# hwwang55/GraphGAN

Measured on AMD Instinct MI355X. Metric: sampled_edges_per_sec, higher is better.
Workload: dtype f32

## Files before the change

### graphgan_amd/_lib.py

```python
from __future__ import annotations

import ctypes
import os

_HERE = os.path.dirname(os.path.abspath(__file__))
LIB_PATH = os.path.join(_HERE, "libgraphgan_hip.so")
HEADER_PATH = os.path.join(os.path.dirname(_HERE), "include", "graphgan_hip.h")
ABI_VERSION = 9


def header_abi_version(path=HEADER_PATH):
    import re
    with open(path) as f:
        m = re.search(r"^#define\s+GG_ABI_VERSION\s+(\d+)", f.read(), flags=re.M)
    if not m:
        raise RuntimeError("GG_ABI_VERSION not found in %s" % path)
    return int(m.group(1))

GG_OK, GG_EINVAL, GG_ECAPACITY, GG_EHIP, GG_ECOMM, GG_ENOMEM, GG_EIO = 0, -1, -2, -3, -4, -5, -6
GG_OPT_ADAM_DENSE, GG_OPT_ADAM_LAZY, GG_OPT_SGD = 0, 1, 2
GG_ROOT_OK, GG_ROOT_ABORTED, GG_ROOT_EMPTY = 0, 1, 2
GG_GS_FOR_D, GG_GS_Q3_STORE = 1, 2
ERROR_NAMES = {GG_EINVAL: "GG_EINVAL", GG_ECAPACITY: "GG_ECAPACITY", GG_EHIP: "GG_EHIP", GG_ECOMM: "GG_ECOMM",
               GG_ENOMEM: "GG_ENOMEM", GG_EIO: "GG_EIO"}


class GGConfig(ctypes.Structure):
    _fields_ = [("lr_gen", ctypes.c_float), ("lr_dis", ctypes.c_float),
                ("lambda_gen", ctypes.c_float), ("lambda_dis", ctypes.c_float),
                ("adam_beta1", ctypes.c_float), ("adam_beta2", ctypes.c_float), ("adam_eps", ctypes.c_float),
                ("window_size", ctypes.c_int32), ("optimizer", ctypes.c_int32), ("device", ctypes.c_int32),
                ("reserved", ctypes.c_int32 * 6)]


class GGCounters(ctypes.Structure):
    _fields_ = [("walks", ctypes.c_int64), ("hops", ctypes.c_int64), ("nbr_reads", ctypes.c_int64),
                ("reward_pairs", ctypes.c_int64), ("d_pairs", ctypes.c_int64), ("g_pairs", ctypes.c_int64),
                ("d_steps", ctypes.c_int64), ("g_steps", ctypes.c_int64),
                ("last_kernel_ms", ctypes.c_double), ("walk_kernel_ms", ctypes.c_double),
                ("walk_launches", ctypes.c_int64), ("rows_scored", ctypes.c_int64), ("score_kernel_ms", ctypes.c_double),
                ("score_launches", ctypes.c_int64), ("score_chunks", ctypes.c_int64), ("score_rows", ctypes.c_int64),
                ("bfs_kernel_ms", ctypes.c_double), ("bfs_trees", ctypes.c_int64), ("score_dists", ctypes.c_int64),
                ("reward_kernel_ms", ctypes.c_double), ("reward_pairs_timed", ctypes.c_int64),
                ("d_grad_ms", ctypes.c_double), ("d_opt_ms", ctypes.c_double), ("d_pairs_timed", ctypes.c_int64), ("d_rows_timed", ctypes.c_int64),
                ("g_grad_ms", ctypes.c_double), ("g_opt_ms", ctypes.c_double), ("g_pairs_timed", ctypes.c_int64), ("g_rows_timed", ctypes.c_int64),
                ("d_passes_timed", ctypes.c_int64), ("g_passes_timed", ctypes.c_int64),
                ("g_walk_nodes_timed", ctypes.c_int64),
                ("es_gathers", ctypes.c_int64), ("es_nodes", ctypes.c_int64), ("score_gathers", ctypes.c_int64), ("score_nodes", ctypes.c_int64),
                ("walk_reruns", ctypes.c_int64)]


class GGGraph(ctypes.Structure):
    _fields_ = [("n_node", ctypes.c_int32), ("nnz", ctypes.c_int64), ("n_train_edges", ctypes.c_int64),
                ("n_test_edges", ctypes.c_int64), ("rowptr", ctypes.POINTER(ctypes.c_int64)), ("col", ctypes.POINTER(ctypes.c_int32))]


class GraphGANHipError(RuntimeError):
    def __init__(self, code, msg):
        super().__init__("%s (%d): %s" % (ERROR_NAMES.get(code, "GG_E?"), code, msg))
        self.code = code


_P = ctypes.c_void_p
_i32, _i64, _u32, _u64 = ctypes.c_int32, ctypes.c_int64, ctypes.c_uint32, ctypes.c_uint64

SIGNATURES = {
    "gg_abi_version": (ctypes.c_int, []),
    "gg_last_error": (ctypes.c_char_p, [_P]),
    "gg_create": (ctypes.c_int, [_i32, _i32, _P, _P, ctypes.POINTER(GGConfig), ctypes.POINTER(_P)]),
    "gg_destroy": (ctypes.c_int, [_P]),
    "gg_set_graph_csr": (ctypes.c_int, [_P, _P, _P]),
    "gg_host_build_trees": (_i64, [_i32, _P, _P, _P, _i32, _P, _P, _P, _i64, _i32, _P]),
    "gg_build_trees": (ctypes.c_int, [_P, _P, _i32, _i32]),
    "gg_build_trees_device": (ctypes.c_int, [_P, _P, _i32]),
    "gg_set_tree_mode": (ctypes.c_int, [_P, _i32, _i64]),
    "gg_debug_words": (ctypes.c_int, [_P, _i32, _i32, _P]),
    "gg_lazy_stats": (ctypes.c_int, [_P, _P]),
    "gg_get_lazy_trees": (ctypes.c_int, [_P, _P, _P, _P, _P, _P, _P, _P]),
    "gg_set_trees": (ctypes.c_int, [_P, _P, _i32, _P, _P, _P, _i32]),
    "gg_tree_info": (ctypes.c_int, [_P, _P, _P, _P]),
    "gg_tree_roots": (ctypes.c_int, [_P, _P]),
    "gg_save_trees": (ctypes.c_int, [_P, ctypes.c_char_p]),
# ... 84 lines not shown
```

### graphgan_amd/csrc/epoch.hip

```cpp
#include <algorithm>
#include <vector>

#include "gg_internal.h"

namespace gg {

int launch_pair_reward(gg_ctx *ctx, const int32_t *d_u, const int32_t *d_v, int64_t n, float *d_out);

__global__ __launch_bounds__(256) void q3_copy_kernel(const int32_t *t_root, const int64_t *t_q3off, uint32_t *t_q3, const int64_t *s_off,
                                                      uint32_t *store, int n_slots, int to_store) {
    const int s = blockIdx.x * blockDim.x + threadIdx.x;
    if (s >= n_slots) return;
    const int v = t_root[s];
    const int64_t a = t_q3off[s], b = s_off[v], words = min(t_q3off[s + 1] - a, s_off[v + 1] - b);
    for (int64_t k = 0; k < words; ++k) {
        if (to_store) store[b + k] = t_q3[a + k];
        else t_q3[a + k] = store[b + k];
    }
}

static int ensure_q3_store(gg_ctx *ctx) {
    if (ctx->q3_store_ready) return GG_OK;
    GG_CHECK(ctx, !ctx->h_rowptr.empty(), GG_EINVAL, "epoch: call gg_set_graph_csr first");
    const int n = ctx->n_node;
// ... 96 lines not shown
        if (rc == GG_OK && do_g) {
            int64_t pairs = 0;
            rc = gg_prepare_g(ctx, slots.data(), n_roots, n_sample, seed, stream_g, &pairs, nullptr);
            if (rc == GG_OK) rc = ensure_g_pairs(ctx);
            if (rc == GG_OK) rc = append(ctx, ctx->ep_node1, ctx->g_node1, ctx->ep_pairs, pairs, sizeof(int32_t));
            if (rc == GG_OK) rc = append(ctx, ctx->ep_node2, ctx->g_node2, ctx->ep_pairs, pairs, sizeof(int32_t));
            if (rc == GG_OK) ctx->ep_pairs += pairs;
        }
        ctx->in_epoch_add = false;
        if (rc != GG_OK) return rc;
        GG_HIP(ctx, hipStreamSynchronize(ctx->stream));
    }
    if (rows_total_out) *rows_total_out = ctx->ep_rows;
    if (pairs_total_out) *pairs_total_out = ctx->ep_pairs;
    return GG_OK;
}

int gg_epoch_commit(gg_ctx *ctx, int32_t which, int64_t *n_out) {
    if (!ctx) return fail(nullptr, GG_EINVAL, "ctx is NULL");
    GG_CHECK(ctx, which == 0 || which == 1, GG_EINVAL, "gg_epoch_commit: which must be 0 (generator pairs) or 1 (discriminator rows)");
    GG_HIP(ctx, hipSetDevice(ctx->device));
    discard_begun_walk(ctx);
    GG_HIP(ctx, hipStreamSynchronize(ctx->stream));
    int rc;
    if (which == 1) {
        const int64_t rows = ctx->ep_rows;
        GG_HIP(ctx, ctx->ep_center.reserve(sizeof(int32_t)));
        GG_HIP(ctx, ctx->ep_neighbor.reserve(sizeof(int32_t)));
        GG_HIP(ctx, ctx->ep_label.reserve(sizeof(float)));
        std::swap(ctx->d_center, ctx->ep_center);
        std::swap(ctx->d_neighbor, ctx->ep_neighbor);
        std::swap(ctx->d_label, ctx->ep_label);
        ctx->d_rows = rows;
        ctx->ep_rows = 0;
        ctx->ep_d_open = false;
        rc = exchange_count_max(ctx, ctx->d_rows, &ctx->d_rows_max);
        if (rc != GG_OK) return rc;
        if (n_out) *n_out = rows;
    } else {
        const int64_t pairs = ctx->ep_pairs;
        GG_HIP(ctx, ctx->ep_node1.reserve(sizeof(int32_t)));
        GG_HIP(ctx, ctx->ep_node2.reserve(sizeof(int32_t)));
        GG_HIP(ctx, ctx->ep_reward.reserve(sizeof(float) * (size_t)(pairs + 1)));
        rc = launch_pair_reward(ctx, ctx->ep_node1.as<int32_t>(), ctx->ep_node2.as<int32_t>(), pairs, ctx->ep_reward.as<float>());
        if (rc != GG_OK) return rc;
        GG_HIP(ctx, hipStreamSynchronize(ctx->stream));
        std::swap(ctx->g_node1, ctx->ep_node1);
        std::swap(ctx->g_node2, ctx->ep_node2);
        std::swap(ctx->g_reward, ctx->ep_reward);
        ctx->g_pairs = pairs;
        ctx->g_pairs_filled = true;
        ctx->g_paths_valid = false;
        ctx->ep_pairs = 0;
        rc = exchange_count_max(ctx, ctx->g_pairs, &ctx->g_pairs_max);
        if (rc != GG_OK) return rc;
        if (n_out) *n_out = pairs;
    }
    return GG_OK;
}

int gg_q3_clear(gg_ctx *ctx) {
    if (!ctx) return fail(nullptr, GG_EINVAL, "ctx is NULL");
    GG_HIP(ctx, hipSetDevice(ctx->device));
    int rc = ensure_q3_store(ctx);
    if (rc != GG_OK) return rc;
    GG_HIP(ctx, hipStreamSynchronize(ctx->stream));
// ... 17 lines not shown
```

### graphgan_amd/csrc/gg_internal.h

```cpp
#pragma once
#include <hip/hip_runtime.h>
#include <stdint.h>
#include <stdio.h>
#include <string>
#include <vector>

#include "../../include/graphgan_hip.h"

namespace gg {

struct DevBuf {
    void *p = nullptr;
    size_t bytes = 0;
    hipError_t reserve(size_t need) {
        if (need <= bytes) return hipSuccess;
        if (p) {
            (void)hipDeviceSynchronize();
            (void)hipFree(p);
        }
        p = nullptr;
        bytes = 0;
        size_t want = need + need / 4 + 256;
        hipError_t e = hipMalloc(&p, want);
        if (e == hipSuccess) bytes = want;
// ... 135 lines not shown
    int tm_cur = -1;

    gg::DevBuf d_center, d_neighbor, d_label, d_cnt, d_ptr;
    int64_t d_rows = 0;
    gg::DevBuf g_node1, g_node2, g_reward, g_cnt, g_ptr;
    int64_t g_pairs = 0;
    bool g_paths_valid = false;
    bool g_begun = false;
    struct { int32_t n_slots = 0, n_sample = 0; uint64_t seed = 0; uint32_t stream = 0; } g_begun_args;
    gg::DevBuf touched_ptr;
    gg::DevBuf bfs_key, bfs_bm, bfs_misc, bfs_sparse, bfs_rowptr32;
    bool bfs_rowptr32_valid = false;
    gg::DevBuf q3_store, q3s_off;
    int64_t q3_words = 0;
    bool q3_store_ready = false;
    gg::DevBuf ep_center, ep_neighbor, ep_label, ep_node1, ep_node2, ep_reward;
    int64_t ep_rows = 0, ep_pairs = 0;
    std::vector<int32_t> ep_slots;
    bool in_epoch_add = false;
    int n_cus = 256;
    gg::DevBuf scan_tmp, step_u, step_v, step_x;
    gg::DevBuf sg_cnt, sg_off, sg_slot, sg_list, sg_rows, sg_bias, sg_tot, sg_key;
    bool g_pairs_filled = false;
    bool sg_cnt_dirty = false;
    gg::DevBuf sgp_cnt, sgp_off, sgp_slot, sgp_list, sgp_tot, sgp_key, sgp_scan, sgp_hub;
    gg::DevBuf sg_hub, hub_acc;
    int64_t hub_cap = 0;
    hipEvent_t ev_slots_done = nullptr;
    bool g_slots_ready = false;
    bool sgp_cnt_clean = false;
    int g_slots_unused = 0;
    int64_t g_slots_walks = 0;
    int32_t g_slots_stride = 0;
    int32_t *sg_cnt_active = nullptr;
    bool sg_active = false;
    int sg_threshold = 64;

    unsigned long long *dev_ctr = nullptr;
    gg_counters ctr{};

    void *comm = nullptr;
    bool comm_rsag = true;
    size_t grad_elems_padded = 0;
    int64_t d_rows_max = 0, g_pairs_max = 0;
    int64_t step_bound = 0;
    int64_t comm_steps_sparse = 0, comm_steps_dense = 0, comm_bytes_sent = 0;
    int32_t rank = 0, world = 1;
    bool deterministic = true;
    float dense_exchange_ratio = 1.5f;
    int32_t fake_world = 0;
    gg::DevBuf x_cnt, x_send_ids, x_send_rows, x_recv_ids, x_recv_rows;
    gg::DevBuf x_nglob;
    gg::DevBuf x_own;
    int32_t owner_exchange = 1;
    bool comm_bf16 = false;
    int64_t owner_min_bound = 4096;
    int64_t comm_steps_owner = 0;

    gg::DevBuf topk_adj;
    bool topk_adj_valid = false;

    gg::DevBuf gs_es, gs_cpre;
    int64_t gs_chunks = 0;
    bool gs_es_valid = false, gs_cpre_valid = false;

    gg::DevBuf pt_starts, pt_paths, pt_len, pt_cnt, pt_ptr, pt_noise, pt_sample;
// ... 23 lines not shown
#define GG_CHECK(ctx, cond, code, ...)                        \
    do {                                                      \
        if (!(cond)) return gg::fail(ctx, code, __VA_ARGS__); \
    } while (0)

int device_exclusive_scan(gg_ctx *ctx, const int32_t *cnt, int64_t *ptr, int64_t n);
int ensure_g_pairs(gg_ctx *ctx);
int device_compact_flags(gg_ctx *ctx, const int32_t *flag, int64_t n, int32_t *list, int64_t *total_out);
int device_segment_rows(gg_ctx *ctx, const int32_t *cnt, int64_t n, int T, int32_t *off, int4 *list, int64_t *totals, hipStream_t stream = nullptr,
                        DevBuf *scratch = nullptr);

int alloc_trees(gg_ctx *ctx, const int32_t *roots, int32_t n_roots, const int64_t *node_counts, const int64_t *root_children, int64_t extra_nodes = 0);
bool lazy_build_wanted(const gg_ctx *ctx);
int lazy_rebuild_whole(gg_ctx *ctx);
int lazy_fallback_rebuild(gg_ctx *ctx, int *n_out);
void component_sizes(int n, const int64_t *rowptr, const int32_t *col, std::vector<int32_t> &comp_size);
int32_t host_bfs_order(const int64_t *rowptr, const int32_t *col, int32_t root, int32_t *order, int32_t *cstart,
                       std::vector<uint32_t> &stamp, uint32_t &epoch, int32_t *depth_out, int32_t *max_children_out);
void order_to_lists(int32_t n, int32_t C, const int32_t *order, const int32_t *cstart, const uint32_t *q3, int32_t *off, int32_t *nbr);
int32_t lists_to_order(int32_t n, int32_t root, const int32_t *off, const int32_t *nbr, int32_t *order, int32_t *cstart,
                       uint32_t *q3, int32_t q3_words, int32_t *depth_out, int32_t *max_children_out);

int walk_launch_async(gg_ctx *ctx, const int32_t *slots, const int32_t *n_walks, int32_t uniform_walks, int32_t n_slots,
                      int32_t for_d, uint64_t seed, uint32_t stream, int32_t stride, bool side_stream = false, bool defer_join = false);
void discard_begun_walk(gg_ctx *ctx);
int walk_finalize(gg_ctx *ctx, bool *retried);
int timing_slot(gg_ctx *ctx);
int check_exchange_flag(gg_ctx *ctx);
void harvest_timings(gg_ctx *ctx);
int derive_tree_edges(gg_ctx *ctx);
int compute_reverse_edges(gg_ctx *ctx);
int rescan_table_finite(gg_ctx *ctx, int which);
int enqueue_path_slots(gg_ctx *ctx);
void generator_changed(gg_ctx *ctx);
int walk_resident(gg_ctx *ctx, const int32_t *slots, const int32_t *n_walks, int32_t uniform_walks, int32_t n_slots,
                  int32_t for_d, uint64_t seed, uint32_t stream, int32_t stride);
int launch_walk_sample(gg_ctx *ctx, int32_t n_slots, int64_t total_walks, int for_d, uint64_t seed, uint32_t stream,
                       int32_t stride);
int run_step(gg_ctx *ctx, int which, const int32_t *d_u, const int32_t *d_v, const float *d_x, int32_t n);
int comm_allreduce_grads(gg_ctx *ctx);
int comm_allreduce_flags(gg_ctx *ctx);
int comm_allreduce_i64(gg_ctx *ctx, int64_t *buf, size_t count);
int comm_allreduce_max_i64(gg_ctx *ctx, int64_t *buf, size_t count);
size_t comm_dense_bytes(const gg_ctx *ctx);
int exchange_count_max(gg_ctx *ctx, int64_t local, int64_t *max_out);
int comm_allgather(gg_ctx *ctx, const void *send, void *recv, size_t count, int elem_bytes);
bool comm_has_p2p(const gg_ctx *ctx);
int comm_exchange_v(gg_ctx *ctx, const float *send, const int64_t *send_off, const int64_t *send_cnt, float *recv, const int64_t *recv_off,
                    const int64_t *recv_cnt);
void comm_destroy(gg_ctx *ctx);

static inline int cdiv(int64_t a, int64_t b) { return (int)((a + b - 1) / b); }

}
```

### graphgan_amd/csrc/prepare.hip

```cpp
#include <algorithm>

#include <cstring>

#include "gg_internal.h"

namespace gg {

constexpr int SCAN_THREADS = 256;
constexpr int SCAN_ITEMS = 8;
constexpr int SCAN_TILE = SCAN_THREADS * SCAN_ITEMS;

__device__ __forceinline__ int64_t block_excl_scan(int64_t v, int64_t *total, int64_t *sh ) {
    const int lane = threadIdx.x & 63, wv = threadIdx.x >> 6;
    int64_t inc = v;
#pragma unroll
    for (int off = 1; off < 64; off <<= 1) {
        const int64_t o = __shfl_up(inc, off, 64);
        if (lane >= off) inc += o;
    }
    if (lane == 63) sh[wv] = inc;
    __syncthreads();
    int64_t base = 0, tot = 0;
#pragma unroll
    for (int i = 0; i < SCAN_THREADS / 64; ++i) {
// ... 384 lines not shown
    if (ctx->g_pairs_filled || ctx->g_pairs == 0) return GG_OK;
    GG_CHECK(ctx, ctx->g_paths_valid, GG_EINVAL,
             "the walks of the last gg_prepare_g were overwritten by a later walk launch before its pairs were read: fetch the pairs "
             "(gg_get_g_data) or run the minibatch passes before the next prepare call");
    return fill_g_pairs(ctx);
}

}

using namespace gg;

extern "C" {

static int enqueue_d_rows(gg_ctx *ctx, int32_t n_slots) {
    hipLaunchKernelGGL(d_count_kernel, dim3(cdiv(n_slots, 256)), dim3(256), 0, ctx->stream, ctx->w_status.as<int32_t>(),
                       ctx->w_ptr_buf().as<int64_t>(), n_slots, ctx->d_cnt.as<int32_t>(), ctx->dev_ctr + 3);
    int rc = device_exclusive_scan(ctx, ctx->d_cnt.as<int32_t>(), ctx->d_ptr.as<int64_t>(), n_slots);
    if (rc != GG_OK) return rc;
    hipLaunchKernelGGL(d_fill_kernel, dim3(cdiv((int64_t)n_slots * 64, 256)), dim3(256), 0, ctx->stream,
                       ctx->w_slots_buf().as<int32_t>(), ctx->t_root, ctx->g_rowptr, ctx->g_col, ctx->w_samples.as<int32_t>(),
                       ctx->w_ptr_buf().as<int64_t>(), ctx->d_ptr.as<int64_t>(), n_slots, ctx->d_center.as<int32_t>(),
                       ctx->d_neighbor.as<int32_t>(), ctx->d_label.as<float>(), ctx->dev_ctr + 3);
    GG_HIP(ctx, hipMemcpyAsync(ctx->h_pin + gg_ctx::H_TOTAL, ctx->d_ptr.as<int64_t>() + n_slots, sizeof(int64_t), hipMemcpyDeviceToHost, ctx->stream));
    GG_HIP(ctx, hipGetLastError());
    return GG_OK;
}

int gg_prepare_d(gg_ctx *ctx, const int32_t *slots, int32_t n_slots, uint64_t seed, uint32_t stream, int64_t *n_rows_out,
                 int32_t *root_status) {
    if (!ctx) return fail(nullptr, GG_EINVAL, "ctx is NULL");
    GG_CHECK(ctx, ctx->g_rowptr, GG_EINVAL, "gg_prepare_d: call gg_set_graph_csr first");
    const int stride = ctx->tree_max_depth + 3;
    ctx->d_rows = 0;
    ctx->dc_valid = false;
    discard_begun_walk(ctx);
    ctx->dc_request = ctx->dc_enabled ? 1 : 0;
    int rc = walk_launch_async(ctx, slots, nullptr, -1, n_slots, 1, seed, stream, stride);
    if (rc != GG_OK) { ctx->dc_request = 0; return rc; }
    if (n_slots > 0) {
        const int64_t cap = 2 * ctx->w_total;
        GG_HIP(ctx, ctx->d_cnt.reserve(sizeof(int32_t) * n_slots));
        GG_HIP(ctx, ctx->d_ptr.reserve(sizeof(int64_t) * (n_slots + 1)));
        GG_HIP(ctx, ctx->d_center.reserve(sizeof(int32_t) * (cap + 1)));
        GG_HIP(ctx, ctx->d_neighbor.reserve(sizeof(int32_t) * (cap + 1)));
        GG_HIP(ctx, ctx->d_label.reserve(sizeof(float) * (cap + 1)));
        rc = enqueue_d_rows(ctx, n_slots);
        if (rc != GG_OK) return rc;
    }
    bool retried = false;
    rc = walk_finalize(ctx, &retried);
    ctx->dc_request = 0;
    if (rc != GG_OK) return rc;
    if (n_slots > 0) {
        if (retried) {
            rc = enqueue_d_rows(ctx, n_slots);
            if (rc != GG_OK) return rc;
            GG_HIP(ctx, hipStreamSynchronize(ctx->stream));
        }
        ctx->d_rows = (int64_t)ctx->h_pin[gg_ctx::H_TOTAL];
        ctx->dc_valid = ctx->dc_enabled && ctx->walk_levels > 0;
        if (root_status) GG_HIP(ctx, hipMemcpy(root_status, ctx->w_status.p, sizeof(int32_t) * n_slots, hipMemcpyDeviceToHost));
    }
    if (!ctx->in_epoch_add) {
        rc = exchange_count_max(ctx, ctx->d_rows, &ctx->d_rows_max);
        if (rc != GG_OK) return rc;
    }
    if (n_rows_out) *n_rows_out = ctx->d_rows;
    return GG_OK;
}

int gg_get_d_data(gg_ctx *ctx, int32_t *center, int32_t *neighbor, float *label) {
    if (!ctx) return fail(nullptr, GG_EINVAL, "ctx is NULL");
    const int64_t n = ctx->d_rows;
    if (n == 0) return GG_OK;
    GG_HIP(ctx, hipSetDevice(ctx->device));
    GG_HIP(ctx, hipStreamSynchronize(ctx->stream));
    if (center) GG_HIP(ctx, hipMemcpy(center, ctx->d_center.p, sizeof(int32_t) * n, hipMemcpyDeviceToHost));
    if (neighbor) GG_HIP(ctx, hipMemcpy(neighbor, ctx->d_neighbor.p, sizeof(int32_t) * n, hipMemcpyDeviceToHost));
    if (label) GG_HIP(ctx, hipMemcpy(label, ctx->d_label.p, sizeof(float) * n, hipMemcpyDeviceToHost));
    return GG_OK;
}

static int enqueue_g_pairs(gg_ctx *ctx, int64_t nw, int64_t cap) {
    const int window = ctx->cfg.window_size;
    hipLaunchKernelGGL(pair_count_kernel, dim3(cdiv(nw, 256)), dim3(256), 0, ctx->stream, ctx->w_len.as<int32_t>(), nw, window,
                       ctx->g_cnt.as<int32_t>(), ctx->dev_ctr + 3);
    int rc = device_exclusive_scan(ctx, ctx->g_cnt.as<int32_t>(), ctx->g_ptr.as<int64_t>(), nw);
    if (rc != GG_OK) return rc;
    const int nch = (ctx->ld / 4 + 15) / 16;
    const bool path_reward = window <= 2 && nch <= 4 && ctx->ld % 4 == 0 && !getenv("GG_NO_PATH_REWARD");
    ctx->g_pairs_filled = false;
    if (!path_reward) {
        rc = fill_g_pairs(ctx);
        if (rc != GG_OK) return rc;
    }
    const Model &D = ctx->model[1];
    const int ts = ctx->walk_timed ? timing_slot(ctx) : -1;
    if (ts >= 0) GG_HIP(ctx, hipEventRecord(ctx->tm_ev[ts][0], ctx->stream));
    if (path_reward) {
// ... 162 lines not shown
```

### graphgan_amd/csrc/pretrain.hip

```cpp
#include <algorithm>
#include <vector>

#include "gg_arith.h"
#include "gg_internal.h"

namespace gg {

constexpr int PT_MAX_LEN = 256, PT_MAX_WINDOW = 16, PT_MAX_NEG = 64;
constexpr int PT_WAVES = 4;
constexpr int PT_SAMPLE = 2048;
constexpr int H_PT_TOTAL = gg_ctx::H_TOTAL + 8;

__host__ __device__ __forceinline__ int pt_pairs_of(int i, int len, int window) {
    const int back = i < window ? i : window, fwd = len - 1 - i < window ? len - 1 - i : window;
    return back + fwd;
}

static int64_t pt_pairs_of_path(int len, int window) {
    int64_t c = 0;
    for (int i = 0; i < len; ++i) c += pt_pairs_of(i, len, window);
    return c;
}

__global__ __launch_bounds__(256) void pt_walk_kernel(const int64_t *__restrict__ rowptr, const int32_t *__restrict__ col,
// ... 143 lines not shown
    std::vector<uint64_t> sample((size_t)ns);
    for (int64_t k = 0; k < ns; ++k) sample[k] = cum[std::min<int64_t>((k + 1) * stride, n) - 1];
    ctx->pt_noise_set = false;
    GG_HIP(ctx, ctx->pt_noise.reserve(sizeof(uint64_t) * (size_t)n));
    GG_HIP(ctx, ctx->pt_sample.reserve(sizeof(uint64_t) * PT_SAMPLE));
    GG_HIP(ctx, hipMemcpy(ctx->pt_noise.p, cum.data(), sizeof(uint64_t) * (size_t)n, hipMemcpyHostToDevice));
    GG_HIP(ctx, hipMemcpy(ctx->pt_sample.p, sample.data(), sizeof(uint64_t) * (size_t)ns, hipMemcpyHostToDevice));
    ctx->pt_noise_total = run;
    ctx->pt_sample_n = (int32_t)ns;
    ctx->pt_sample_stride = (int32_t)stride;
    ctx->pt_noise_set = true;
    return GG_OK;
}

int gg_prepare_pretrain(gg_ctx *ctx, const int32_t *starts, int32_t n_starts, int32_t walks_per_start, int32_t walk_len,
                        int32_t window, int32_t n_neg, uint64_t seed, uint32_t stream, int64_t *n_rows_out, int32_t *paths,
                        int32_t *path_len) {
    if (!ctx) return fail(nullptr, GG_EINVAL, "ctx is NULL");
    GG_CHECK(ctx, ctx->g_rowptr, GG_EINVAL, "gg_prepare_pretrain: call gg_set_graph_csr first");
    GG_CHECK(ctx, !ctx->comm, GG_EINVAL, "gg_prepare_pretrain: a communicator is attached (pre-training is single rank)");
    GG_CHECK(ctx, !ctx->ep_d_open, GG_EINVAL, "gg_prepare_pretrain: called between gg_epoch_begin and gg_epoch_commit(1)");
    GG_CHECK(ctx, n_starts >= 0 && (starts || n_starts == 0), GG_EINVAL, "gg_prepare_pretrain: bad starts");
    GG_CHECK(ctx, walks_per_start >= 1, GG_EINVAL, "gg_prepare_pretrain: walks_per_start must be >= 1");
    GG_CHECK(ctx, walk_len >= 1 && walk_len <= PT_MAX_LEN, GG_EINVAL, "gg_prepare_pretrain: walk_len must be in [1, %d]", PT_MAX_LEN);
    GG_CHECK(ctx, window >= 1 && window <= PT_MAX_WINDOW, GG_EINVAL, "gg_prepare_pretrain: window must be in [1, %d]", PT_MAX_WINDOW);
    GG_CHECK(ctx, n_neg >= 0 && n_neg <= PT_MAX_NEG, GG_EINVAL, "gg_prepare_pretrain: n_neg must be in [0, %d]", PT_MAX_NEG);
    GG_CHECK(ctx, ctx->n_node >= 3, GG_EINVAL, "gg_prepare_pretrain: the collision rule of the negatives needs n_node >= 3");
    for (int32_t i = 0; i < n_starts; ++i)
        GG_CHECK(ctx, starts[i] >= 0 && starts[i] < ctx->n_node, GG_EINVAL, "gg_prepare_pretrain: starts[%d] = %d out of range", i, starts[i]);
    const int64_t nw = (int64_t)n_starts * walks_per_start;
    GG_CHECK(ctx, nw <= 0x7fffffffll, GG_ECAPACITY, "gg_prepare_pretrain: %lld walks in one call", (long long)nw);
    GG_HIP(ctx, hipSetDevice(ctx->device));
    ctx->d_rows = 0;
    if (nw > 0) {
        const int64_t rows_bound = nw * (1 + n_neg) * pt_pairs_of_path(walk_len, window);
        const bool sized = rows_bound <= 0x7fffffffll;
        GG_HIP(ctx, ctx->pt_starts.reserve(sizeof(int32_t) * (size_t)n_starts));
        GG_HIP(ctx, ctx->pt_paths.reserve(sizeof(int32_t) * (size_t)nw * walk_len));
        GG_HIP(ctx, ctx->pt_len.reserve(sizeof(int32_t) * (size_t)nw));
        GG_HIP(ctx, ctx->pt_cnt.reserve(sizeof(int32_t) * (size_t)nw));
        GG_HIP(ctx, ctx->pt_ptr.reserve(sizeof(int64_t) * (size_t)(nw + 1)));
        const bool timed = ctx->profile_every == 1;
        if (timed && !ctx->pt_ev[0])
            for (hipEvent_t &e : ctx->pt_ev) GG_HIP(ctx, hipEventCreate(&e));
        GG_HIP(ctx, hipMemcpyAsync(ctx->pt_starts.p, starts, sizeof(int32_t) * (size_t)n_starts, hipMemcpyHostToDevice, ctx->stream));
        if (timed) GG_HIP(ctx, hipEventRecord(ctx->pt_ev[0], ctx->stream));
        hipLaunchKernelGGL(pt_walk_kernel, dim3(cdiv(nw, 256)), dim3(256), 0, ctx->stream, ctx->g_rowptr, ctx->g_col,
                           ctx->pt_starts.as<int32_t>(), nw, walks_per_start, walk_len, seed, stream, ctx->pt_paths.as<int32_t>(),
                           ctx->pt_len.as<int32_t>());
        if (timed) GG_HIP(ctx, hipEventRecord(ctx->pt_ev[1], ctx->stream));
        hipLaunchKernelGGL(pt_count_kernel, dim3(cdiv(nw, 256)), dim3(256), 0, ctx->stream, ctx->pt_len.as<int32_t>(), nw, window, n_neg,
                           ctx->pt_cnt.as<int32_t>());
        GG_HIP(ctx, hipGetLastError());
        int rc = device_exclusive_scan(ctx, ctx->pt_cnt.as<int32_t>(), ctx->pt_ptr.as<int64_t>(), nw);
        if (rc != GG_OK) return rc;
        GG_HIP(ctx, hipMemcpyAsync(ctx->h_pin + H_PT_TOTAL, ctx->pt_ptr.as<int64_t>() + nw, sizeof(int64_t), hipMemcpyDeviceToHost, ctx->stream));
        int64_t cap = rows_bound;
        if (!sized) {
            GG_HIP(ctx, hipStreamSynchronize(ctx->stream));
            cap = (int64_t)ctx->h_pin[H_PT_TOTAL];
            GG_CHECK(ctx, cap <= 0x7fffffffll, GG_ECAPACITY, "gg_prepare_pretrain: %lld rows in one call (at most 2^31 - 1): pass fewer starts",
                     (long long)cap);
        }
        GG_HIP(ctx, ctx->d_center.reserve(sizeof(int32_t) * (size_t)(cap + 1)));
        GG_HIP(ctx, ctx->d_neighbor.reserve(sizeof(int32_t) * (size_t)(cap + 1)));
        GG_HIP(ctx, ctx->d_label.reserve(sizeof(float) * (size_t)(cap + 1)));
// ... 34 lines not shown
```

### graphgan_amd/csrc/steps.hip

```cpp
#include <stdlib.h>

#include <algorithm>
#include <cmath>
#include <vector>

#include "gg_internal.h"

namespace gg {

struct HubAcc {
    unsigned long long *acc;
    int64_t cap;
    float scale;
};
__device__ __forceinline__ unsigned long long *hub_row(const HubAcc &h, int slot, int ld) {
    const int64_t k = -3 - (int64_t)slot;
    return (slot <= -3 && k < h.cap) ? h.acc + k * (ld + 1) : nullptr;
}
__device__ __forceinline__ void hub_add(unsigned long long *p, float x, float scale) {
    atomicAdd(p, (unsigned long long)__float2ll_rn(x * scale));
}

struct StepArgs {
    float *E, *b;
// ... 1110 lines not shown
        const int f = (int)(i - h * (ld + 1));
        const float x = (float)((double)(long long)v * inv_scale);
        if (f < ld) gE[(int64_t)rows[h] * ld + f] += x;
        else gb[rows[h]] += x;
    }
}

static float hub_scale(bool per_pair_mean, int64_t n) {
    return std::ldexp(1.0f, 32 + (per_pair_mean && n > 1 ? (int)std::ilogb((double)n) : 0));
}

static HubAcc hub_args(gg_ctx *ctx, float scale) {
    return HubAcc{ctx->hub_acc.as<unsigned long long>(), ctx->hub_cap, scale};
}

static int hub_index(gg_ctx *ctx, const int32_t *cnt, int32_t *off, DevBuf &rows, int64_t *tot, hipStream_t stream) {
    GG_HIP(ctx, rows.reserve(sizeof(int32_t) * (size_t)ctx->n_node));
    GG_HIP(ctx, hipMemsetAsync(tot + 2, 0, sizeof(int64_t), stream));
    hipLaunchKernelGGL(hub_index_kernel, dim3((unsigned)cdiv(ctx->n_node, 256)), dim3(256), 0, stream, cnt, (int64_t)ctx->n_node, ctx->sg_threshold, off,
                       rows.as<int32_t>(), tot + 2);
    GG_HIP(ctx, hipGetLastError());
    return GG_OK;
}

static void hub_finalize(gg_ctx *ctx, bool early_index, float scale, float *gE, float *gb) {
    DevBuf &rows = early_index ? ctx->sgp_hub : ctx->sg_hub, &tot = early_index ? ctx->sgp_tot : ctx->sg_tot;
    const int64_t n = ctx->hub_cap * (ctx->ld + 1);
    const unsigned nb = (unsigned)std::max<int64_t>(1, std::min<int64_t>(cdiv(n, 256), 2048));
    hipLaunchKernelGGL(hub_finalize_kernel, dim3(nb), dim3(256), 0, ctx->stream, ctx->hub_acc.as<unsigned long long>(), rows.as<int32_t>(),
                       tot.as<int64_t>() + 2, ctx->hub_cap, ctx->ld, 1.0 / (double)scale, gE, gb);
}

static int staged_reserve(gg_ctx *ctx, int64_t n_occ, int64_t n_stage) {
    if (n_stage * (int64_t)(ctx->ld + 2) * 4 > stage_bytes_cap()) return 1;
    const size_t cnt_before = ctx->sg_cnt.bytes;
    GG_HIP(ctx, ctx->sg_cnt.reserve(sizeof(int32_t) * (size_t)ctx->n_node));
    const bool was_dirty = ctx->sg_cnt_dirty;
    if (ctx->sg_cnt.bytes != cnt_before || ctx->sg_cnt_dirty) GG_HIP(ctx, hipMemsetAsync(ctx->sg_cnt.p, 0, ctx->sg_cnt.bytes, ctx->stream));
    ctx->sg_cnt_dirty = true;
    GG_HIP(ctx, ctx->sg_off.reserve(sizeof(int32_t) * (size_t)ctx->n_node));
    GG_HIP(ctx, ctx->sg_list.reserve(sizeof(int4) * (size_t)ctx->n_node));
    GG_HIP(ctx, ctx->sg_slot.reserve(sizeof(int32_t) * (size_t)n_occ));
    GG_HIP(ctx, ctx->sg_bias.reserve(sizeof(float) * (size_t)n_stage));
    GG_HIP(ctx, ctx->sg_key.reserve(sizeof(int32_t) * (size_t)n_stage));
    GG_HIP(ctx, ctx->sg_tot.reserve(sizeof(int64_t) * 4));
    {
        const int64_t cap = std::min<int64_t>(ctx->n_node, n_occ / ((int64_t)ctx->sg_threshold + 1) + 1);
        const size_t before = ctx->hub_acc.bytes;
        if (ctx->hub_acc.reserve(sizeof(unsigned long long) * (size_t)cap * (ctx->ld + 1)) != hipSuccess) {
            (void)hipGetLastError();
            ctx->hub_cap = 0;
            return 1;
        }
        if (ctx->hub_acc.bytes != before || was_dirty) GG_HIP(ctx, hipMemsetAsync(ctx->hub_acc.p, 0, ctx->hub_acc.bytes, ctx->stream));
        ctx->hub_cap = (int64_t)(ctx->hub_acc.bytes / (sizeof(unsigned long long) * (ctx->ld + 1)));
    }
    if (ctx->sg_rows.reserve(sizeof(float) * (size_t)n_stage * ctx->ld) != hipSuccess) {
        (void)hipGetLastError();
        return 1;
    }
    return GG_OK;
}

static int staged_finish(gg_ctx *ctx, int which, int64_t n, int64_t n_occ, bool early_index = false) {
    const int opt = ctx->cfg.optimizer;
    OptArgs o = make_opt_args(ctx, which);
    DevBuf &b_cnt = early_index ? ctx->sgp_cnt : ctx->sg_cnt, &b_list = early_index ? ctx->sgp_list : ctx->sg_list;
    DevBuf &b_tot = early_index ? ctx->sgp_tot : ctx->sg_tot, &b_key = early_index ? ctx->sgp_key : ctx->sg_key;
    o.sg_cnt = b_cnt.as<int32_t>(); o.sg_list = b_list.as<int4>(); o.sg_tot = b_tot.as<int64_t>();
    o.stage = ctx->sg_rows.as<float>(); o.stage_b = ctx->sg_bias.as<float>(); o.stage_key = b_key.as<int32_t>();
    int nb = cdiv((int64_t)std::min<int64_t>(n_occ, ctx->n_node) * 16, 256);
    if (nb > 4096) nb = 4096;
    if (nb < 1) nb = 1;
    const bool replicas = ctx->comm || ctx->fake_world > 1;
    if (replicas) hipLaunchKernelGGL(staged_opt_kernel<2>, dim3(nb), dim3(256), 0, ctx->stream, o);
    else if (opt == GG_OPT_SGD) hipLaunchKernelGGL(staged_opt_kernel<1>, dim3(nb), dim3(256), 0, ctx->stream, o);
    else hipLaunchKernelGGL(staged_opt_kernel<0>, dim3(nb), dim3(256), 0, ctx->stream, o);
    ctx->sg_active = true;
    ctx->sg_cnt_active = o.sg_cnt;
    const int rc = apply_optimizer(ctx, which, n);
    ctx->sg_active = false;
    if (rc != GG_OK) return rc;
    if (!replicas)
        hipLaunchKernelGGL(add_word_kernel, dim3(1), dim3(1), 0, ctx->stream, ctx->touched_ptr.as<int64_t>() + ctx->n_node, b_tot.as<int64_t>());
    GG_HIP(ctx, hipGetLastError());
    if (early_index) ctx->sgp_cnt_clean = true;
    else ctx->sg_cnt_dirty = false;
    return GG_OK;
}

static bool staged_allowed(const gg_ctx *ctx) {
    return ctx->sg_threshold > 0 && ctx->ld <= 256 && ctx->cfg.optimizer != GG_OPT_ADAM_DENSE && !getenv("GG_NO_STAGED_GRAD");
}

int run_step(gg_ctx *ctx, int which, const int32_t *d_u, const int32_t *d_v, const float *d_x, int32_t n) {
    if (n <= 0) return GG_OK;
    Model &M = ctx->model[which];
    const int opt = ctx->cfg.optimizer;
    StepArgs s{};
    s.E = M.E; s.b = M.b; s.gE = ctx->gradE; s.gb = ctx->gradb;
    s.touched = ctx->touched; s.touched_list = ctx->touched_list; s.touched_cnt = ctx->touched_cnt;
    s.ld = ctx->ld;
    s.track = opt != GG_OPT_ADAM_DENSE;
    s.u = d_u; s.v = d_v; s.x = d_x; s.n = n;
    s.lambda = M.lambda;
    s.inv_n = 1.0f / (float)n;
    s.is_d = which == 1;
    if (which == 0) {
        int rc = global_pair_count(ctx, n, &s.n_glob);
        if (rc != GG_OK) return rc;
    }
    s.ppg = n >= 16384 ? PAIRS_PER_GROUP : (n >= 2048 ? 4 : 1);
    if (ctx->deterministic && n <= DET_MAX_PAIRS) {
        const int nfd = (ctx->ld + 15) / 16;
        const bool replicas = ctx->comm || ctx->fake_world > 1;
        const int fused = (!replicas && opt != GG_OPT_ADAM_DENSE && det_rows_fit_lds(ctx, s) && !getenv("GG_NO_FUSED_SMALL_STEP")) ? (opt == GG_OPT_SGD ? 2 : 1) : 0;
        const OptArgs o = make_opt_args(ctx, which);
        static unsigned long long *det_prof = nullptr;
        static const bool det_prof_on = getenv("GG_DET_PROFILE") != nullptr;
        if (det_prof_on) {
            if (!det_prof) GG_HIP(ctx, hipMalloc((void **)&det_prof, 16 * sizeof(unsigned long long)));
            GG_HIP(ctx, hipMemsetAsync(det_prof, 0, 16 * sizeof(unsigned long long), ctx->stream));
            s.prof = det_prof;
        }
        hipError_t e;
        if (nfd <= 4) e = launch_pair_grad_det<4>(ctx, s, o, fused);
        else if (nfd <= 8) e = launch_pair_grad_det<8>(ctx, s, o, fused);
        else if (nfd <= 16) e = launch_pair_grad_det<16>(ctx, s, o, fused);
        else e = launch_pair_grad_det<32>(ctx, s, o, fused);
        GG_HIP(ctx, e);
        if (det_prof_on) {
            static double acc_t[2][2][4] = {};
            static long cnt[2] = {};
            unsigned long long h[16];
            GG_HIP(ctx, hipMemcpyAsync(h, det_prof, sizeof(h), hipMemcpyDeviceToHost, ctx->stream));
            GG_HIP(ctx, hipStreamSynchronize(ctx->stream));
            for (int w = 0; w < 2; ++w)
                for (int k = 0; k < 3; ++k) acc_t[which][w][k] += h[8 * w + k + 1] > h[8 * w + k] ? 10.0 * (double)(h[8 * w + k + 1] - h[8 * w + k]) : 0.0;
            if (++cnt[which] % 1000 == 0)
                for (int w = 0; w < 2; ++w)
                    fprintf(stderr, "[det] model %d n=%d wave %s: loads+coef %.0f ns, barrier %.0f, owners' sums + stores issued %.0f (means over %ld steps)\n", which, n, w ? "15" : "0",
                            acc_t[which][w][0] / cnt[which], acc_t[which][w][1] / cnt[which], acc_t[which][w][2] / cnt[which], cnt[which]);
        }
        if (fused) {
            GG_HIP(ctx, hipGetLastError());
            step_done(ctx, which, n);
            return GG_OK;
        }
        return apply_optimizer(ctx, which, n);
    }
    const int groups = cdiv(n, s.ppg);
    const int blocks = cdiv((int64_t)groups * 16, 256);
    const int nf = (ctx->ld + 15) / 16;
    bool staged = n >= 16384 && n < (1 << 30) && staged_allowed(ctx);
    if (staged) {
        int rc = staged_reserve(ctx, 2 * (int64_t)n, 2 * (int64_t)n);
        if (rc < 0) return rc;
        if (rc == 1) staged = false;
    }
    if (staged) {
        int rc;
        int32_t *cnt = ctx->sg_cnt.as<int32_t>(), *off = ctx->sg_off.as<int32_t>(), *slot_v = ctx->sg_slot.as<int32_t>(), *slot_u = slot_v + n;
        hipLaunchKernelGGL(pair_occ_count_kernel, dim3(cdiv(n, 256)), dim3(256), 0, ctx->stream, d_u, d_v, n, s.ppg, cnt, slot_v, slot_u);
        rc = device_segment_rows(ctx, cnt, ctx->n_node, ctx->sg_threshold, off, ctx->sg_list.as<int4>(), ctx->sg_tot.as<int64_t>());
        if (rc != GG_OK) return rc;
        rc = hub_index(ctx, cnt, off, ctx->sg_hub, ctx->sg_tot.as<int64_t>(), ctx->stream);
        if (rc != GG_OK) return rc;
        hipLaunchKernelGGL(pair_occ_slot_kernel, dim3(cdiv(n, 256)), dim3(256), 0, ctx->stream, d_u, d_v, n, cnt, off, ctx->sg_threshold, slot_v, slot_u,
                           ctx->sg_key.as<int32_t>());
        s.slot_v = slot_v; s.slot_u = slot_u;
        s.stage = ctx->sg_rows.as<float>(); s.stage_b = ctx->sg_bias.as<float>();
        const float scale = hub_scale(!s.is_d, n);
        s.hub = hub_args(ctx, scale);
        if (nf <= 4) hipLaunchKernelGGL((pair_grad16_kernel<4, true>), dim3(blocks), dim3(256), 0, ctx->stream, s);
        else if (nf <= 8) hipLaunchKernelGGL((pair_grad16_kernel<8, true>), dim3(blocks), dim3(256), 0, ctx->stream, s);
        else hipLaunchKernelGGL((pair_grad16_kernel<16, true>), dim3(blocks), dim3(256), 0, ctx->stream, s);
        hub_finalize(ctx, false, scale, s.gE, s.gb);
        if (ctx->tm_cur >= 0) GG_HIP(ctx, hipEventRecord(ctx->tm_ev[ctx->tm_cur][1], ctx->stream));
        return staged_finish(ctx, which, n, 2 * (int64_t)n);
    }
    if (s.ppg == PAIRS_PER_GROUP && nf <= 16 && !getenv("GG_OLD_PAIR_GRAD")) {
        if (nf <= 4) hipLaunchKernelGGL((pair_grad16_kernel<4, false>), dim3(blocks), dim3(256), 0, ctx->stream, s);
        else if (nf <= 8) hipLaunchKernelGGL((pair_grad16_kernel<8, false>), dim3(blocks), dim3(256), 0, ctx->stream, s);
        else hipLaunchKernelGGL((pair_grad16_kernel<16, false>), dim3(blocks), dim3(256), 0, ctx->stream, s);
    } else if (nf <= 4) hipLaunchKernelGGL((pair_grad_kernel<4, false>), dim3(blocks), dim3(256), 0, ctx->stream, s);
    else if (nf <= 8) hipLaunchKernelGGL((pair_grad_kernel<8, false>), dim3(blocks), dim3(256), 0, ctx->stream, s);
    else if (nf <= 16) hipLaunchKernelGGL((pair_grad_kernel<16, false>), dim3(blocks), dim3(256), 0, ctx->stream, s);
    else hipLaunchKernelGGL((pair_grad_kernel<32, false>), dim3(blocks), dim3(256), 0, ctx->stream, s);
    if (ctx->tm_cur >= 0) GG_HIP(ctx, hipEventRecord(ctx->tm_ev[ctx->tm_cur][1], ctx->stream));

    return apply_optimizer(ctx, which, n);
}

template <bool STAGED>
static void launch_path_grad(gg_ctx *ctx, const PathArgs &p, int blocks, int nf) {
    const dim3 g(blocks), b(256);
    if (p.stride <= 17) {
        if (nf <= 4) hipLaunchKernelGGL((path_grad_kernel<4, STAGED, true>), g, b, 0, ctx->stream, p);
        else if (nf <= 8) hipLaunchKernelGGL((path_grad_kernel<8, STAGED, true>), g, b, 0, ctx->stream, p);
        else hipLaunchKernelGGL((path_grad_kernel<16, STAGED, true>), g, b, 0, ctx->stream, p);
    } else {
        if (nf <= 4) hipLaunchKernelGGL((path_grad_kernel<4, STAGED, false>), g, b, 0, ctx->stream, p);
// ... 76 lines not shown
    if (ctx->g_slots_unused >= 2) {
        if (ctx->sgp_slot.p) {
            for (DevBuf *b : {&ctx->sgp_cnt, &ctx->sgp_off, &ctx->sgp_slot, &ctx->sgp_list, &ctx->sgp_key, &ctx->sgp_scan, &ctx->sgp_hub}) b->release();
            ctx->sgp_cnt_clean = false;
        }
        return GG_OK;
    }
    hipStream_t st = ctx->walk_stream;
    const size_t cnt_before = ctx->sgp_cnt.bytes;
    GG_HIP(ctx, ctx->sgp_cnt.reserve(sizeof(int32_t) * (size_t)ctx->n_node));
    if (ctx->sgp_cnt.bytes != cnt_before || !ctx->sgp_cnt_clean) GG_HIP(ctx, hipMemsetAsync(ctx->sgp_cnt.p, 0, ctx->sgp_cnt.bytes, st));
    ctx->sgp_cnt_clean = false;
    GG_HIP(ctx, ctx->sgp_off.reserve(sizeof(int32_t) * (size_t)ctx->n_node));
    GG_HIP(ctx, ctx->sgp_list.reserve(sizeof(int4) * (size_t)ctx->n_node));
    GG_HIP(ctx, ctx->sgp_slot.reserve(sizeof(int32_t) * (size_t)n_pos));
    GG_HIP(ctx, ctx->sgp_key.reserve(sizeof(int32_t) * (size_t)n_pos));
    GG_HIP(ctx, ctx->sgp_tot.reserve(sizeof(int64_t) * 4));
    if (!ctx->ev_slots_done) GG_HIP(ctx, hipEventCreateWithFlags(&ctx->ev_slots_done, hipEventDisableTiming));
    const unsigned long long *flag = ctx->dev_ctr + 3;
    const dim3 pgrid((unsigned)cdiv(n_pos, 256));
    int32_t *cnt = ctx->sgp_cnt.as<int32_t>(), *off = ctx->sgp_off.as<int32_t>(), *slot = ctx->sgp_slot.as<int32_t>();
    hipLaunchKernelGGL(path_count_kernel, pgrid, dim3(256), 0, st, ctx->w_paths.as<int32_t>(), ctx->w_len.as<int32_t>(), ctx->w_stride, n_walks, cnt, slot, flag);
    int rc = device_segment_rows(ctx, cnt, ctx->n_node, ctx->sg_threshold, off, ctx->sgp_list.as<int4>(), ctx->sgp_tot.as<int64_t>(), st, &ctx->sgp_scan);
    if (rc != GG_OK) return rc;
    rc = hub_index(ctx, cnt, off, ctx->sgp_hub, ctx->sgp_tot.as<int64_t>(), st);
    if (rc != GG_OK) return rc;
    hipLaunchKernelGGL(path_slot_kernel, pgrid, dim3(256), 0, st, ctx->w_paths.as<int32_t>(), ctx->w_len.as<int32_t>(), ctx->w_stride, n_walks, cnt, off,
                       ctx->sg_threshold, slot, ctx->sgp_key.as<int32_t>(), flag);
    GG_HIP(ctx, hipGetLastError());
    GG_HIP(ctx, hipEventRecord(ctx->ev_slots_done, st));
    ctx->g_slots_ready = true;
    ctx->g_slots_walks = n_walks;
    ctx->g_slots_stride = ctx->w_stride;
    return GG_OK;
}

__global__ void normalize_flags_kernel(int32_t *f, int n) {
    const int i = blockIdx.x * blockDim.x + threadIdx.x;
    if (i < n && f[i] > 1) f[i] = 1;
}

__global__ void scale_grads_kernel(float *gE, float *gb, int64_t nE, int n, float k) {
    const int64_t stride = (int64_t)gridDim.x * blockDim.x;
    for (int64_t i = (int64_t)blockIdx.x * blockDim.x + threadIdx.x; i < nE; i += stride) gE[i] *= k;
    for (int64_t i = (int64_t)blockIdx.x * blockDim.x + threadIdx.x; i < n; i += stride) gb[i] *= k;
}

__global__ __launch_bounds__(256) void owner_count_kernel(const int32_t *list, const int64_t *cnt_ptr, int world, long long *cnt) {
    __shared__ int sh[64];
    if (threadIdx.x < 64) sh[threadIdx.x] = 0;
    __syncthreads();
    const int64_t n = *cnt_ptr;
    for (int64_t i = (int64_t)blockIdx.x * blockDim.x + threadIdx.x; i < n; i += (int64_t)gridDim.x * blockDim.x) atomicAdd(&sh[list[i] % world], 1);
    __syncthreads();
    if ((int)threadIdx.x < world && sh[threadIdx.x]) atomicAdd((unsigned long long *)&cnt[threadIdx.x], (unsigned long long)sh[threadIdx.x]);
}

template <bool BF16>
__global__ __launch_bounds__(256) void owner_pack_kernel(const float *gE, const float *gb, const int32_t *list, const int64_t *cnt_ptr, int world,
                                                         const long long *seg_off, long long *fill, int ld, int32_t *out_ids, float *out_rows) {
    const int t = threadIdx.x & 15;
    const int64_t g0 = ((int64_t)blockIdx.x * blockDim.x + threadIdx.x) >> 4, ng = ((int64_t)gridDim.x * blockDim.x) >> 4;
    const int64_t cnt = *cnt_ptr;
    for (int64_t r = g0; r < cnt; r += ng) {
        const int row = list[r];
        const int q = row % world;
// ... 449 lines not shown
```

### include/graphgan_hip.h

```cpp
#ifndef GRAPHGAN_HIP_H
#define GRAPHGAN_HIP_H

#include <stdint.h>

#ifdef __cplusplus
extern "C" {
#endif

#define GG_ABI_VERSION 9

enum {
    GG_OK = 0,
    GG_EINVAL = -1,
    GG_ECAPACITY = -2,
    GG_EHIP = -3,
    GG_ECOMM = -4,
    GG_ENOMEM = -5,
    GG_EIO = -6
};

enum {
    GG_OPT_ADAM_DENSE = 0,
    GG_OPT_ADAM_LAZY = 1,
    GG_OPT_SGD = 2
// ... 22 lines not shown
typedef struct gg_counters {
    int64_t walks;
    int64_t hops;
    int64_t nbr_reads;
    int64_t reward_pairs;
    int64_t d_pairs;
    int64_t g_pairs;
    int64_t d_steps;
    int64_t g_steps;
    double last_kernel_ms;
    double walk_kernel_ms;
    int64_t walk_launches;
    int64_t rows_scored;
    double score_kernel_ms;
    int64_t score_launches;
    int64_t score_chunks;
    int64_t score_rows;
    double bfs_kernel_ms;
    int64_t bfs_trees;
    int64_t score_dists;
    double reward_kernel_ms;
    int64_t reward_pairs_timed;
    double d_grad_ms, d_opt_ms;
    int64_t d_pairs_timed, d_rows_timed;
    double g_grad_ms, g_opt_ms;
    int64_t g_pairs_timed, g_rows_timed;
    int64_t d_passes_timed, g_passes_timed;
    int64_t g_walk_nodes_timed;
    int64_t es_gathers;
    int64_t es_nodes;
    int64_t score_gathers;
    int64_t score_nodes;
    int64_t walk_reruns;
} gg_counters;

typedef struct gg_ctx gg_ctx;

int gg_abi_version(void);
const char *gg_last_error(const gg_ctx *ctx);

int gg_create(int32_t n_node, int32_t n_emb, const float *emb_gen, const float *emb_dis,
              const gg_config *cfg, gg_ctx **out);
int gg_destroy(gg_ctx *ctx);

int gg_set_graph_csr(gg_ctx *ctx, const int64_t *rowptr , const int32_t *col);

int64_t gg_host_build_trees(int32_t n_node, const int64_t *rowptr, const int32_t *col,
                            const int32_t *roots, int32_t n_roots,
                            int32_t *off , int32_t *nbr, int64_t *nbr_base ,
                            int64_t cap, int32_t n_threads, int32_t *max_depth_out);

int gg_build_trees(gg_ctx *ctx, const int32_t *roots, int32_t n_roots, int32_t n_threads);
int gg_build_trees_device(gg_ctx *ctx, const int32_t *roots, int32_t n_roots);
int gg_set_tree_mode(gg_ctx *ctx, int32_t mode, int64_t node_cap);
int gg_debug_words(gg_ctx *ctx, int32_t first, int32_t n, uint64_t *out);
int gg_lazy_stats(gg_ctx *ctx, int64_t *out24);
int gg_get_lazy_trees(gg_ctx *ctx, int64_t *n_entries, int32_t *info4, int64_t *base, int32_t *order, int32_t *cstart, int32_t *edge, uint64_t *pair);
int gg_set_trees(gg_ctx *ctx, const int32_t *roots, int32_t n_roots, const int32_t *off,
                 const int32_t *nbr, const int64_t *nbr_base, int32_t max_depth);
int gg_tree_info(const gg_ctx *ctx, int32_t *n_roots, int64_t *n_entries, int32_t *max_depth);
int gg_tree_roots(const gg_ctx *ctx, int32_t *roots );
int gg_save_trees(gg_ctx *ctx, const char *path);
int gg_load_trees(gg_ctx *ctx, const char *path);
int gg_get_trees(gg_ctx *ctx, int32_t *off, int32_t *nbr, int64_t *nbr_base);
int gg_get_tree_order(gg_ctx *ctx, int64_t *base, int32_t *order, int32_t *cstart, int32_t *edge, int32_t *edges_valid);

// ... 106 lines not shown
```

Before: 661.3 million.

## Build discriminator pair-occupancy index at prepare time and reuse in first D step

Moves construction of the staged-gradient pair index (count, segment, hub index, slot kernels) for discriminator rows from the first training step into gg_prepare_d, keyed by buffer pointers, a generation counter, optimizer and threshold. The first D step then skips rebuilding the index when the key matches. The aim is to take index building off the step's critical path and overlap it with preparation work. It adds invalidation state and a fallback that releases staged buffers after repeated unused builds, plus counters for built and used indexes.

```diff
diff --git a/graphgan_amd/_lib.py b/graphgan_amd/_lib.py
--- a/graphgan_amd/_lib.py
+++ b/graphgan_amd/_lib.py
@@ -47,7 +47,8 @@
                 ("d_passes_timed", ctypes.c_int64), ("g_passes_timed", ctypes.c_int64),
                 ("g_walk_nodes_timed", ctypes.c_int64),
                 ("es_gathers", ctypes.c_int64), ("es_nodes", ctypes.c_int64), ("score_gathers", ctypes.c_int64), ("score_nodes", ctypes.c_int64),
-                ("walk_reruns", ctypes.c_int64)]
+                ("walk_reruns", ctypes.c_int64),
+                ("d_slots_built", ctypes.c_int64), ("d_slots_used", ctypes.c_int64)]
 
 
 class GGGraph(ctypes.Structure):
diff --git a/graphgan_amd/csrc/epoch.hip b/graphgan_amd/csrc/epoch.hip
--- a/graphgan_amd/csrc/epoch.hip
+++ b/graphgan_amd/csrc/epoch.hip
@@ -152,6 +152,7 @@
         std::swap(ctx->d_neighbor, ctx->ep_neighbor);
         std::swap(ctx->d_label, ctx->ep_label);
         ctx->d_rows = rows;
+        d_rows_changed(ctx);
         ctx->ep_rows = 0;
         ctx->ep_d_open = false;
         rc = exchange_count_max(ctx, ctx->d_rows, &ctx->d_rows_max);
diff --git a/graphgan_amd/csrc/gg_internal.h b/graphgan_amd/csrc/gg_internal.h
--- a/graphgan_amd/csrc/gg_internal.h
+++ b/graphgan_amd/csrc/gg_internal.h
@@ -191,6 +191,12 @@
     int g_slots_unused = 0;
     int64_t g_slots_walks = 0;
     int32_t g_slots_stride = 0;
+    bool d_slots_ready = false;
+    bool d_slots_pending = false;
+    bool d_slots_own_alloc = false;
+    int d_slots_unused = 0;
+    uint64_t d_gen = 0;
+    struct { const int32_t *u = nullptr, *v = nullptr; int32_t n = 0; uint64_t gen = 0; int32_t optimizer = 0, threshold = 0; } d_slots_key;
     int32_t *sg_cnt_active = nullptr;
     bool sg_active = false;
     int sg_threshold = 64;
@@ -280,6 +286,8 @@
 int compute_reverse_edges(gg_ctx *ctx);
 int rescan_table_finite(gg_ctx *ctx, int which);
 int enqueue_path_slots(gg_ctx *ctx);
+int enqueue_d_slots(gg_ctx *ctx);
+static inline void d_rows_changed(gg_ctx *ctx) { ctx->d_gen++; ctx->d_slots_ready = false; }
 void generator_changed(gg_ctx *ctx);
 int walk_resident(gg_ctx *ctx, const int32_t *slots, const int32_t *n_walks, int32_t uniform_walks, int32_t n_slots,
                   int32_t for_d, uint64_t seed, uint32_t stream, int32_t stride);
diff --git a/graphgan_amd/csrc/prepare.hip b/graphgan_amd/csrc/prepare.hip
--- a/graphgan_amd/csrc/prepare.hip
+++ b/graphgan_amd/csrc/prepare.hip
@@ -440,6 +440,7 @@
     GG_CHECK(ctx, ctx->g_rowptr, GG_EINVAL, "gg_prepare_d: call gg_set_graph_csr first");
     const int stride = ctx->tree_max_depth + 3;
     ctx->d_rows = 0;
+    d_rows_changed(ctx);
     ctx->dc_valid = false;
     discard_begun_walk(ctx);
     ctx->dc_request = ctx->dc_enabled ? 1 : 0;
@@ -473,6 +474,8 @@
         rc = exchange_count_max(ctx, ctx->d_rows, &ctx->d_rows_max);
         if (rc != GG_OK) return rc;
     }
+    rc = enqueue_d_slots(ctx);
+    if (rc != GG_OK) return rc;
     if (n_rows_out) *n_rows_out = ctx->d_rows;
     return GG_OK;
 }
diff --git a/graphgan_amd/csrc/pretrain.hip b/graphgan_amd/csrc/pretrain.hip
--- a/graphgan_amd/csrc/pretrain.hip
+++ b/graphgan_amd/csrc/pretrain.hip
@@ -199,6 +199,7 @@
     GG_CHECK(ctx, nw <= 0x7fffffffll, GG_ECAPACITY, "gg_prepare_pretrain: %lld walks in one call", (long long)nw);
     GG_HIP(ctx, hipSetDevice(ctx->device));
     ctx->d_rows = 0;
+    d_rows_changed(ctx);
     if (nw > 0) {
         const int64_t rows_bound = nw * (1 + n_neg) * pt_pairs_of_path(walk_len, window);
         const bool sized = rows_bound <= 0x7fffffffll;
diff --git a/graphgan_amd/csrc/steps.hip b/graphgan_amd/csrc/steps.hip
--- a/graphgan_amd/csrc/steps.hip
+++ b/graphgan_amd/csrc/steps.hip
@@ -1166,6 +1166,8 @@
 }
 
 static int staged_reserve(gg_ctx *ctx, int64_t n_occ, int64_t n_stage) {
+    ctx->d_slots_ready = false;
+    ctx->d_slots_own_alloc = false;
     if (n_stage * (int64_t)(ctx->ld + 2) * 4 > stage_bytes_cap()) return 1;
     const size_t cnt_before = ctx->sg_cnt.bytes;
     GG_HIP(ctx, ctx->sg_cnt.reserve(sizeof(int32_t) * (size_t)ctx->n_node));
@@ -1227,6 +1229,21 @@
     return ctx->sg_threshold > 0 && ctx->ld <= 256 && ctx->cfg.optimizer != GG_OPT_ADAM_DENSE && !getenv("GG_NO_STAGED_GRAD");
 }
 
+static int enqueue_pair_index(gg_ctx *ctx, const int32_t *d_u, const int32_t *d_v, int32_t n, int ppg) {
+    int32_t *cnt = ctx->sg_cnt.as<int32_t>(), *off = ctx->sg_off.as<int32_t>(), *slot_v = ctx->sg_slot.as<int32_t>(), *slot_u = slot_v + n;
+    hipLaunchKernelGGL(pair_occ_count_kernel, dim3(cdiv(n, 256)), dim3(256), 0, ctx->stream, d_u, d_v, n, ppg, cnt, slot_v, slot_u);
+    int rc = device_segment_rows(ctx, cnt, ctx->n_node, ctx->sg_threshold, off, ctx->sg_list.as<int4>(), ctx->sg_tot.as<int64_t>());
+    if (rc != GG_OK) return rc;
+    rc = hub_index(ctx, cnt, off, ctx->sg_hub, ctx->sg_tot.as<int64_t>(), ctx->stream);
+    if (rc != GG_OK) return rc;
+    hipLaunchKernelGGL(pair_occ_slot_kernel, dim3(cdiv(n, 256)), dim3(256), 0, ctx->stream, d_u, d_v, n, cnt, off, ctx->sg_threshold, slot_v, slot_u,
+                       ctx->sg_key.as<int32_t>());
+    GG_HIP(ctx, hipGetLastError());
+    return GG_OK;
+}
+
+static bool staged_batch(const gg_ctx *ctx, int64_t n) { return n >= 16384 && n < (1 << 30) && staged_allowed(ctx); }
+
 int run_step(gg_ctx *ctx, int which, const int32_t *d_u, const int32_t *d_v, const float *d_x, int32_t n) {
     if (n <= 0) return GG_OK;
     Model &M = ctx->model[which];
@@ -1286,22 +1303,28 @@
     const int groups = cdiv(n, s.ppg);
     const int blocks = cdiv((int64_t)groups * 16, 256);
     const int nf = (ctx->ld + 15) / 16;
-    bool staged = n >= 16384 && n < (1 << 30) && staged_allowed(ctx);
-    if (staged) {
+    bool staged = staged_batch(ctx, n);
+    const bool fused_d = staged && which == 1 && n == ctx->d_rows && d_u == ctx->d_center.as<int32_t>() && d_v == ctx->d_neighbor.as<int32_t>();
+    if (fused_d) ctx->d_slots_unused = 0;
+    const auto &dk = ctx->d_slots_key;
+    const bool early = fused_d && ctx->d_slots_ready && dk.u == d_u && dk.v == d_v && dk.n == n && dk.gen == ctx->d_gen && dk.optimizer == opt &&
+                       dk.threshold == ctx->sg_threshold && !getenv("GG_NO_EARLY_D_SLOTS");
+    if (early) {
+        ctx->d_slots_ready = false;
+        ctx->d_slots_pending = false;
+        ctx->d_slots_own_alloc = false;
+        ctx->ctr.d_slots_used += 1;
+    } else if (staged) {
         int rc = staged_reserve(ctx, 2 * (int64_t)n, 2 * (int64_t)n);
         if (rc < 0) return rc;
         if (rc == 1) staged = false;
     }
     if (staged) {
-        int rc;
-        int32_t *cnt = ctx->sg_cnt.as<int32_t>(), *off = ctx->sg_off.as<int32_t>(), *slot_v = ctx->sg_slot.as<int32_t>(), *slot_u = slot_v + n;
-        hipLaunchKernelGGL(pair_occ_count_kernel, dim3(cdiv(n, 256)), dim3(256), 0, ctx->stream, d_u, d_v, n, s.ppg, cnt, slot_v, slot_u);
-        rc = device_segment_rows(ctx, cnt, ctx->n_node, ctx->sg_threshold, off, ctx->sg_list.as<int4>(), ctx->sg_tot.as<int64_t>());
-        if (rc != GG_OK) return rc;
-        rc = hub_index(ctx, cnt, off, ctx->sg_hub, ctx->sg_tot.as<int64_t>(), ctx->stream);
-        if (rc != GG_OK) return rc;
-        hipLaunchKernelGGL(pair_occ_slot_kernel, dim3(cdiv(n, 256)), dim3(256), 0, ctx->stream, d_u, d_v, n, cnt, off, ctx->sg_threshold, slot_v, slot_u,
-                           ctx->sg_key.as<int32_t>());
+        int32_t *slot_v = ctx->sg_slot.as<int32_t>(), *slot_u = slot_v + n;
+        if (!early) {
+            int rc = enqueue_pair_index(ctx, d_u, d_v, n, s.ppg);
+            if (rc != GG_OK) return rc;
+        }
         s.slot_v = slot_v; s.slot_u = slot_u;
         s.stage = ctx->sg_rows.as<float>(); s.stage_b = ctx->sg_bias.as<float>();
         const float scale = hub_scale(!s.is_d, n);
@@ -1444,6 +1467,38 @@
     ctx->g_slots_ready = true;
     ctx->g_slots_walks = n_walks;
     ctx->g_slots_stride = ctx->w_stride;
+    return GG_OK;
+}
+
+int enqueue_d_slots(gg_ctx *ctx) {
+    if (ctx->d_slots_pending) {
+        ctx->d_slots_pending = false;
+        ctx->d_slots_unused++;
+    }
+    ctx->d_slots_ready = false;
+    const int64_t n = ctx->d_rows;
+    if (ctx->in_epoch_add || getenv("GG_NO_EARLY_D_SLOTS") || !staged_batch(ctx, n)) return GG_OK;
+    if (ctx->d_slots_unused >= 2) {
+        if (ctx->d_slots_own_alloc) {
+            for (DevBuf *b : {&ctx->sg_cnt, &ctx->sg_off, &ctx->sg_slot, &ctx->sg_list, &ctx->sg_rows, &ctx->sg_bias, &ctx->sg_key, &ctx->sg_hub, &ctx->hub_acc}) b->release();
+            ctx->hub_cap = 0;
+            ctx->d_slots_own_alloc = false;
+        }
+        return GG_OK;
+    }
+    const bool own_alloc = ctx->d_slots_own_alloc || !ctx->sg_rows.p;
+    int rc = staged_reserve(ctx, 2 * n, 2 * n);
+    if (rc < 0) return rc;
+    ctx->d_slots_own_alloc = own_alloc;
+    if (rc == 1) return GG_OK;
+    const int32_t *d_u = ctx->d_center.as<int32_t>(), *d_v = ctx->d_neighbor.as<int32_t>();
+    rc = enqueue_pair_index(ctx, d_u, d_v, (int32_t)n, PAIRS_PER_GROUP);
+    if (rc != GG_OK) return rc;
+    ctx->d_slots_key.u = d_u; ctx->d_slots_key.v = d_v; ctx->d_slots_key.n = (int32_t)n; ctx->d_slots_key.gen = ctx->d_gen;
+    ctx->d_slots_key.optimizer = ctx->cfg.optimizer; ctx->d_slots_key.threshold = ctx->sg_threshold;
+    ctx->d_slots_ready = true;
+    ctx->d_slots_pending = true;
+    ctx->ctr.d_slots_built += 1;
     return GG_OK;
 }
 
diff --git a/include/graphgan_hip.h b/include/graphgan_hip.h
--- a/include/graphgan_hip.h
+++ b/include/graphgan_hip.h
@@ -78,6 +78,8 @@
     int64_t score_gathers;
     int64_t score_nodes;
     int64_t walk_reruns;
+    int64_t d_slots_built;
+    int64_t d_slots_used;
 } gg_counters;
 
 typedef struct gg_ctx gg_ctx;
```

Measured after the change: 631.1 million. 4.6% lower.
